# osmocom/osmo-gmr

Hardware: AMD Instinct MI355X
Metric: Mbursts/s demod+Viterbi (and IQ Msamp/s), 1/2/4/8 MI355X (higher is better)
Workload: dtype f32+i32

## Files before the change

osmo-gmr_amd/csrc/conv_k5_12.h:

```cpp
#pragma once
#include "l1_codes.h"
#include "rx4_operands.h"
#include "wave_ops.h"

namespace gmr1 {

__constant__ StepTable c_steps = make_steps();
__device__ const Rx4Steps4 g_steps4 = make_steps4(make_steps());

struct CostTable { uint32_t a[512], b[512]; };
static constexpr CostTable make_cost()
{
	CostTable t{};
	for (int idx = 0; idx < 512; idx++) {
		int v = (int)(int8_t)(uint8_t)(idx & 255);
		if (idx & 256)
			v = (int)(int8_t)(uint8_t)(-v);
		const int e0 = v - 127, e1 = v + 127;
		const uint32_t c0 = v ? (uint32_t)((e0 * e0) >> 9) : 0u;
		const uint32_t c1 = v ? (uint32_t)((e1 * e1) >> 9) : 0u;
		t.a[idx] = c0 | (c0 << 8) | (c1 << 16) | (c1 << 24);
		t.b[idx] = c0 | (c1 << 8) | (c0 << 16) | (c1 << 24);
	}
	return t;
}
__constant__ CostTable c_cost = make_cost();

static constexpr CostTable make_cost_acc()
{
	CostTable t{};
	for (int idx = 0; idx < 512; idx++) {
		int v = (int)(int8_t)(uint8_t)(idx & 255);
		if (idx & 256)
			v = (int)(int8_t)(uint8_t)(-v);
		const uint32_t c0 = v < 0 ? (uint32_t)(-v) : 0u;
		const uint32_t c1 = v > 0 ? (uint32_t)v : 0u;
		t.a[idx] = c0 | (c0 << 8) | (c1 << 16) | (c1 << 24);
		t.b[idx] = c0 | (c1 << 8) | (c0 << 16) | (c1 << 24);
	}
	return t;
}
__constant__ CostTable c_cost_acc = make_cost_acc();
constexpr uint32_t kAccLeadK5r2 = 127u * 2u * 5u / 2u;

struct SynTable { uint16_t s[208]; };
static constexpr SynTable make_syn()
{
	SynTable t{};
	for (int k = 0; k < 192; k++)
		t.s[k] = (uint16_t)l1c::crc_unit(l1c::kCrc16, k, 192);
	for (int i = 0; i < 16; i++)
		t.s[192 + i] = (uint16_t)(1u << (15 - i));
	return t;
}
__constant__ SynTable c_syn = make_syn();

struct SynRows { uint32_t w[16][8]; };
static constexpr SynRows make_syn_rows()
{
	const SynTable t = make_syn();
	SynRows r{};
	for (int loc = 0; loc < 16; loc++)
		for (int q = 0; q < 13; q++)
			r.w[loc][q >> 1] |= (uint32_t)t.s[13 * loc + q] << (16 * (q & 1));
	return r;
}
__constant__ __attribute__((aligned(16))) SynRows c_syn_rows = make_syn_rows();

struct SbLut { uint16_t v[1024]; };
static constexpr SbLut make_sb_lut()
{
	SbLut t{};
	for (int k = 0; k < 1024; k++) {
		int q = 2 * k + 1;
		if (q > 1024)
			q -= 2048;
		const int n = (q + 256 + 2048) / 512 - 4;
		const int dlq = 512 * n - q;
		const int adl = dlq < 0 ? -dlq : dlq;
		const int dq = (adl + 2) / 4;
		const unsigned sp = (unsigned)n & 3u;
		const unsigned neg = dlq < 0 ? 1u : 0u;
		const bool f0 = ((sp ^ neg ^ 1u) & 1u) != 0;
		const int m_near = 127 - dq, m_far = 127 - (dq >> 1);
		int v0 = f0 ? m_near : m_far;
		int v1 = f0 ? m_far : m_near;
		if (sp >> 1)
			v0 = -v0;
		if ((sp ^ (sp >> 1)) & 1u)
			v1 = -v1;
		t.v[k] = (uint16_t)(((unsigned)v0 & 0xffu) | (((unsigned)v1 & 0xffu) << 8));
	}
	return t;
}
__device__ __attribute__((aligned(16))) const SbLut g_sb_lut = make_sb_lut();
constexpr int kSbLutBytes = 2048;

static constexpr SbLut make_sb_lut1()
{
	SbLut t{};
	for (int k = 0; k < 1024; k++) {
		int q = 2 * k + 1;
		if (q > 1024)
			q -= 2048;
		const int n = (q + 512 + 2048) / 1024 - 2;
		const int dlq = 1024 * n - q;
		const int adl = dlq < 0 ? -dlq : dlq;
		const int dq = (adl + 4) / 8;
		const unsigned sp = (unsigned)n & 1u;
		const int v0 = sp ? -(127 - dq) : (127 - dq);
		t.v[k] = (uint16_t)((unsigned)v0 & 0xffu);
	}
	return t;
}
__device__ __attribute__((aligned(16))) const SbLut g_sb_lut1 = make_sb_lut1();

__device__ __forceinline__ uint32_t out_k5_12(uint32_t s, uint32_t b)
{
	constexpr uint32_t g0 = l1c::kK5_12[0], g1 = l1c::kK5_12[1];
	uint32_t reg = (s << 1) | b;
	return ((uint32_t)(__popc(reg & g0) & 1) << 1) | (uint32_t)(__popc(reg & g1) & 1);
}
__device__ __forceinline__ uint32_t rotl4(uint32_t x, int r) { return ((x << r) | (x >> (4 - r))) & 15u; }

template <bool ACC = false>
__device__ __forceinline__ void branch_metrics_k5_12(const int8_t *__restrict__ eb, int chain,
                                                     uint32_t *__restrict__ bm, int lane)
{
	const CostTable &ct = ACC ? c_cost_acc : c_cost;
	for (int k = lane; k < kSteps12; k += 64) {
		const uint32_t st = c_steps.w[chain][k];
		const uint32_t ia = (uint32_t)(uint8_t)eb[st & 0x3ffu] | ((st >> 2) & 0x100u);
		const uint32_t ib = (uint32_t)(uint8_t)eb[(st >> 16) & 0x3ffu] | ((st >> 18) & 0x100u);
		bm[k] = ct.a[ia] + ct.b[ib];
	}
}

template <bool ACC, class Steps>
__device__ __forceinline__ void branch_metrics4_k5_12_from(const int8_t *__restrict__ eb, int eb_stride, int row_ok,
                                                           int row_chain, uint32_t *__restrict__ bm, int lane, Steps steps)
{
	const CostTable &ct = ACC ? c_cost_acc : c_cost;
	uint32_t st[2][4];
#pragma unroll
	for (int c = 0; c < 2; c++)
#pragma unroll
		for (int it = 0; it < 4; it++)
			st[c][it] = steps(c, it);
	uint32_t ia[4][4], ib[4][4];
#pragma unroll
	for (int q = 0; q < 4; q++) {
		const bool ch = ((row_chain >> q) & 1) != 0;
		const int8_t *e = eb + q * eb_stride;
#pragma unroll
		for (int it = 0; it < 4; it++) {
			const uint32_t s = ch ? st[1][it] : st[0][it];
			ia[q][it] = (uint32_t)(uint8_t)e[s & 0x3ffu] | ((s >> 2) & 0x100u);
			ib[q][it] = (uint32_t)(uint8_t)e[(s >> 16) & 0x3ffu] | ((s >> 18) & 0x100u);
		}
	}
	uint32_t va[4][4], vb[4][4];
#pragma unroll
	for (int q = 0; q < 4; q++)
#pragma unroll
		for (int it = 0; it < 4; it++) {
			va[q][it] = ct.a[ia[q][it]];
			vb[q][it] = ct.b[ib[q][it]];
		}
#pragma unroll
	for (int q = 0; q < 4; q++) {
		const bool ok = ((row_ok >> q) & 1) != 0;
#pragma unroll
		for (int it = 0; it < 4; it++) {
			const int k = lane + 64 * it;
			if (k < kSteps12)
				bm[q * kSteps12 + k] = ok ? va[q][it] + vb[q][it] : 0u;
		}
	}
}

template <bool ACC = false>
__device__ __forceinline__ void branch_metrics4_k5_12(const int8_t *__restrict__ eb, int eb_stride, int row_ok,
                                                      int row_chain, uint32_t *__restrict__ bm, int lane)
{
	branch_metrics4_k5_12_from<ACC>(eb, eb_stride, row_ok, row_chain, bm, lane, [&](int c, int it) -> uint32_t {
		const int k = lane + 64 * it;
		return k < kSteps12 ? c_steps.w[c][k] : 0u;
	});
}

template <bool ACC = false>
__device__ __forceinline__ void branch_metrics4_k5_12(const int8_t *__restrict__ eb, int eb_stride, int row_ok,
                                                      int row_chain, uint32_t *__restrict__ bm, int lane,
                                                      const uint4 st0, const uint4 st1)
{
	branch_metrics4_k5_12_from<ACC>(eb, eb_stride, row_ok, row_chain, bm, lane, [&](int c, int it) -> uint32_t {
		const uint4 v = c ? st1 : st0;
		return it == 0 ? v.x : (it == 1 ? v.y : (it == 2 ? v.z : v.w));
	});
}

constexpr uint32_t kSentinel = 0xF0000000u;

struct DecTable { uint32_t v[16]; };
static constexpr uint32_t dec_out(uint32_t s, uint32_t b)
{
	return l1c::conv_word(l1c::kK5_12, (s << 1) | b);
}
static constexpr uint32_t dec_state(uint32_t loc, int ph)
{
	uint32_t c[4] = {0, 0, 0, 0};
	c[0] = (loc >> 3) & 1u;
	uint32_t x = loc & 7u;
	c[1] = (x >> 2) & 1u;
	x ^= c[1] ? 7u : 0u;
	c[2] = (x >> 1) & 1u;
	c[3] = x & 1u;
	uint32_t sp = 0;
	for (int i = 0; i < 4; i++)
		sp |= c[(3 - i + ph) & 3] << i;
	return sp;
}
static constexpr DecTable make_dec()
{
	DecTable t{};
	for (uint32_t loc = 0; loc < 16; loc++) {
		uint32_t e = 0;
		for (int ph = 0; ph < 4; ph++) {
			const uint32_t sp = dec_state(loc, ph);
			const uint32_t b = sp >> 3;
			e |= dec_out(sp, b) << (2 * ph);
			e |= dec_out(sp, b ^ 1u) << (8 + 2 * ph);
			for (int j = ph; j < 16; j += 4)
				e |= b << (16 + j);
		}
		t.v[loc] = e;
	}
	return t;
}
static constexpr bool dec_exchange_holds()
{
	const DecTable t = make_dec();
	const uint32_t mask[4] = {8u, 7u, 2u, 1u};
	for (uint32_t loc = 0; loc < 16; loc++)
		for (int ph = 0; ph < 4; ph++) {
			const uint32_t sp = dec_state(loc, ph);
			const uint32_t partner_into_mine = dec_out(sp ^ 8u, sp >> 3);
			if (dec_state(loc ^ mask[ph], ph) != (sp ^ 8u))
				return false;
			if (((t.v[loc ^ mask[ph]] >> (8 + 2 * ph)) & 3u) != partner_into_mine)
				return false;
			if (((t.v[loc] >> (8 + 2 * ph)) & 3u) != partner_into_mine)
// ... 374 lines not shown
```

osmo-gmr_amd/csrc/rx4_operands.h:

```cpp
#pragma once
#include <stdint.h>

#include "gmr1_dev.h"
#include "l1_codes.h"

namespace gmr1 {

static constexpr int kSteps12 = 212;

struct StepTable { uint32_t w[2][kSteps12]; };
static constexpr StepTable make_steps()
{
	StepTable t{};
	const auto scr = l1c::scramble_seq<448>();
	for (int chain = 0; chain < 2; chain++) {
		const int off = chain ? 4 : 0;
		for (int k = 0; k < kSteps12; k++) {
			uint32_t w = 0;
			for (int j = 0; j < 2; j++) {
				const int kc = 2 * k + j;
				const int ei = l1c::intra_pos(53, kc) + off;
				w |= ((uint32_t)ei | (scr.bit[ei] ? 0x400u : 0u)) << (16 * j);
			}
			t.w[chain][k] = w;
// ... 7 lines not shown
struct alignas(16) Rx4Steps4 { uint32_t w[2][64][4]; };
static constexpr Rx4Steps4 make_steps4(const StepTable &st)
{
	Rx4Steps4 t{};
	for (int chain = 0; chain < 2; chain++)
		for (int lane = 0; lane < 64; lane++)
			for (int it = 0; it < 4; it++) {
				const int k = lane + 64 * it;
				t.w[chain][lane][it] = k < kSteps12 ? st.w[chain][k] : 0u;
			}
	return t;
}

struct alignas(8) Rx4Ord4 { int16_t v[2][64][4]; };
inline void make_ord4(const DevBurst types[kNumTypes], Rx4Ord4 *out)
{
	for (int kind = 0; kind < 2; kind++) {
		const DevBurst &bt = types[kRx4Type[kind]];
		for (int lane = 0; lane < 64; lane++)
			for (int r = 0; r < 4; r++) {
				const int i = lane + 64 * r;
				out->v[kind][lane][r] = (i < bt.len && i < kMaxLen) ? bt.ord_of_sym[i] : (int16_t)-1;
			}
	}
}

inline bool rx4_ord4_matches(const DevBurst types[kNumTypes], const Rx4Ord4 &o)
{
	for (int kind = 0; kind < 2; kind++) {
		const DevBurst &bt = types[kRx4Type[kind]];
		if (bt.len > 256)
			return false;
		for (int lane = 0; lane < 64; lane++)
			for (int r = 0; r < 4; r++) {
				const int i = lane + 64 * r;
				if (o.v[kind][lane][r] != (i < bt.len ? bt.ord_of_sym[i] : (int16_t)-1))
					return false;
			}
	}
	return true;
}
inline bool rx4_steps4_matches(const StepTable &st, const Rx4Steps4 &s)
{
	for (int chain = 0; chain < 2; chain++)
		for (int lane = 0; lane < 64; lane++)
			for (int it = 0; it < 4; it++) {
				const int k = lane + 64 * it;
				if (s.w[chain][lane][it] != (k < kSteps12 ? st.w[chain][k] : 0u))
					return false;
			}
	return true;
}

}
```

osmo-gmr_amd/csrc/rx_kernels.hip:

```cpp
#include <mutex>
#include <type_traits>

#include "gmr1_dev.h"
#include "tch3_body.h"
#include "wave_ops.h"
#include "fast_math.h"

namespace gmr1 {
__constant__ DevBurst c_types[kNumTypes];
}

#include "conv_k5_12.h"
#include "rx_window.h"

namespace gmr1 {

__device__ Rx4Ord4 g_ord4;

#include "rx_one.h"

__device__ __forceinline__ float2 sync_coef0(const DevBurst &bt, int n, int sps, float fs)
{
	const int nch = bt.n_chunks[0];
	int ch = 0, base = 0, cum = 0;
// ... 360 lines not shown
	const DevBurst &bt = c_types[kind ? GMR1_HIP_DC6 : GMR1_HIP_BCCH];
	const int w = in_len - 234 * sps + 1;
	const float2 *__restrict__ in = a.iq + off;
	constexpr int NFULL = (SPS == 4 && NPL == 16) ? 15 : -1;
	constexpr int SIT = SPS == 4 ? 2 : 4;
	float2 wv[NPL];
	float2 sv[3][SIT];
	window_fetch<NPL, NFULL>(in, in_len, lane, wv);
#pragma unroll
	for (int c = 0; c < 3; c++) {
		const int wl = F::clen(bt, kind, c) * sps + w - 1;
		const float2 *__restrict__ src = in + F::cpos(bt, c) * sps;
#pragma unroll
		for (int h = 0; h < SIT; h++) {
			const int sidx = lane + 64 * h;
			sv[c][h] = sidx < wl ? src[sidx] : make_float2(0.f, 0.f);
		}
	}
	if (win) {
#pragma unroll
		for (int k = 0; k < NPL; k++)
			win[lane + 64 * k] = wv[k];
	}
	float avr, avi, inv;
	window_stats<NPL, NFULL>(wv, in_len, lane, avr, avi, inv);
	const float e = window_energy_regs<NPL>(wv, in_len, lane);
	int wb = 0;
#pragma unroll
	for (int c = 0; c < 3; c++) {
		const int wl = F::clen(bt, kind, c) * sps + w - 1;
#pragma unroll
		for (int h = 0; h < SIT; h++) {
			const int sidx = lane + 64 * h;
			if (sidx < wl) {
				const v2f nv = ((v2f){sv[c][h].x, sv[c][h].y} - (v2f){avr, avi}) * (v2f){inv, inv};
				hx[wb + sidx] = make_float2(nv.x, nv.y);
			}
		}
		wb += wl;
	}
	if (lane == 0) {
		hs[0] = avr;
		hs[1] = avi;
		hs[2] = inv;
		hs[3] = e;
	}
}

struct Rx4Cfg {
	static constexpr int NPL = 16, SPS = 4;
	static constexpr bool LAT = false, GEN = false, FAC = false, ACC = false, EN = true, PL = false;
	static constexpr int EBROW = 432, PART = 0;
	static constexpr bool EARLY = false;
};
template <int NPL_, int SPS_, bool ACC_, bool EN_, bool PL_ = false, bool EARLY_ = false>
struct CfgBatch : Rx4Cfg {
	static constexpr int NPL = NPL_, SPS = SPS_;
	static constexpr bool ACC = ACC_, EN = EN_, PL = PL_, EARLY = EARLY_;
};
template <int NPL_, int SPS_, bool FAC_>
struct CfgDemod : Rx4Cfg {
	static constexpr int NPL = NPL_, SPS = SPS_;
	static constexpr bool GEN = true, FAC = FAC_;
};
struct CfgTch3Front : Rx4Cfg {
	static constexpr int NPL = 8, SPS = 4, EBROW = 216;
	static constexpr bool GEN = true;
};
template <int NPL_, int SPS_, bool ACC_, int PART_ = 0>
struct CfgLoop : Rx4Cfg {
	static constexpr int NPL = NPL_, SPS = SPS_, PART = PART_;
	static constexpr bool LAT = true, ACC = ACC_;
};

#ifndef GMR1_EXP_RX4_TOUCH
#define GMR1_EXP_RX4_TOUCH 0
#endif

template <class P>
struct Rx4Switches : P {
	static constexpr bool SMALL = P::GEN && P::NPL == 8;
	static_assert(!P::FAC || SMALL, "the two-sequence variant builds on the small generic one");
	static_assert(!P::PL || (P::SPS == 4 && !P::GEN && !P::LAT && !P::EN), "the planar layout exists for the fused batch kernel at sps 4");
	static_assert(P::PART == 0 || P::LAT, "only the receive loop's burst is cut in two");
	static constexpr bool PREFETCH_NEXT = P::GEN || P::LAT;
	static constexpr int NSYM = SMALL ? 2 : 4;
	static constexpr int NCHK = SMALL ? 1 : 3;
	static constexpr int NSH = SMALL ? 1 : 2;
	static constexpr bool UB_OVER = !P::LAT && !P::GEN;
	static constexpr bool QL = !P::GEN && !P::LAT && !P::EN && P::SPS == 4 && P::NPL == 16;
	static constexpr bool QX = QL && !P::PL;
	static_assert(!P::PL || QL, "the planar layout exists for the fused batch kernel");
	static constexpr bool AHEAD = P::EARLY && QX;
	static constexpr int TOUCH = AHEAD ? GMR1_EXP_RX4_TOUCH : 0;
	static constexpr bool H_ROW = AHEAD, ONE_LOAD = AHEAD;
	static constexpr bool OPS_AHEAD = AHEAD;
};

constexpr int kRx4StepsAt = 1;

template <class Cfg>
__device__ __forceinline__ void rx4_body(const RxArgs &a, const RxIo io, int stage_samples, int cw, int g0, int n_end,
                                         unsigned char *__restrict__ lds_raw, int lane, LatPre<Cfg::NPL, Cfg::SPS> *pre = nullptr)
{
	typedef Rx4Switches<Cfg> C;
	constexpr int NPL = C::NPL, SPS = C::SPS, EBROW = C::EBROW, PART = C::PART;
	constexpr bool LAT = C::LAT, GEN = C::GEN, FAC = C::FAC, ACC = C::ACC, EN = C::EN, PL = C::PL;
	constexpr bool SMALL = C::SMALL, QL = C::QL, QX = C::QX, PREFETCH_NEXT = C::PREFETCH_NEXT, UB_OVER = C::UB_OVER;
	constexpr int NSYM = C::NSYM, NCHK = C::NCHK, NSH = C::NSH;
	constexpr int TOUCH = C::TOUCH;
	constexpr bool AHEAD = C::AHEAD, H_ROW = C::H_ROW, OPS_AHEAD = C::OPS_AHEAD;
	const int row = lane >> 4, col = lane & 15;
	const int sps = SPS ? SPS : a.sps;
	const int cwh = FAC ? cw / 2 : cw;
	size_t off[4];
	lds4_layout(stage_samples, cw, off, GEN, UB_OVER, EBROW);
	Lds4 L;
	L.x = reinterpret_cast<float2 *>(lds_raw + off[0]);
	L.corr = reinterpret_cast<float *>(lds_raw + off[1]);
	L.coef = reinterpret_cast<float2 *>(lds_raw + off[2]);
	L.eb = reinterpret_cast<int8_t *>(lds_raw + off[3]);
	L.bm = reinterpret_cast<uint32_t *>(lds_raw + off[0]);
	L.surv = reinterpret_cast<uint64_t *>(lds_raw + off[3]);
	L.ubits = reinterpret_cast<uint32_t *>(lds_raw + off[0] + (UB_OVER ? 0 : 4 * kSteps12 * 4));

	const int g_row = g0 + row;
	const bool row_live = g_row < n_end;

	float avr_r = 0.f, avi_r = 0.f;
	const float2 *xst_lat = L.x;

	float th_q[QX ? 4 : 1][4];
	uint32_t zm_q = 0xff000000u;
	float2 xs_q[2] = {make_float2(0.f, 0.f), make_float2(0.f, 0.f)};
	float inv_r = 1.0f;
	auto op_kind = [&](int g) -> int {
		if constexpr (LAT && PART != 0) return 0; else return io.kind[g] ? 1 : 0;
	};
	auto op_fsh = [&](int g) -> float {
		if constexpr (LAT && PART != 0) return pre->b_fsh; else return io.freq_shift ? io.freq_shift[g] : 0.0f;
	};
	auto op_off = [&](int g) -> uint64_t {
		if constexpr (LAT && PART != 0) return pre->b_off; else return io.offset[g];
	};
	int kind_s[4] = {0, 0, 0, 0};
	uint64_t off_s[4] = {0, 0, 0, 0};
	float fsh_s[4] = {0.f, 0.f, 0.f, 0.f};
	if constexpr (AHEAD) {
		if (g0 < n_end) {
			int kv[4];
			uint64_t ov[4];
			float fv[4];
#pragma unroll
			for (int q = 0; q < 4; q++) {
				const int gq = g0 + q < n_end ? g0 + q : g0;
				kv[q] = op_kind(gq);
				ov[q] = op_off(gq);
				fv[q] = op_fsh(gq);
			}
#pragma unroll
			for (int q = 0; q < 4; q++) {
				kind_s[q] = __builtin_amdgcn_readfirstlane(kv[q]);
				off_s[q] = (uint64_t)(uint32_t)__builtin_amdgcn_readfirstlane((int)(uint32_t)ov[q]) |
				           ((uint64_t)(uint32_t)__builtin_amdgcn_readfirstlane((int)(uint32_t)(ov[q] >> 32)) << 32);
				fsh_s[q] = __builtin_bit_cast(float, __builtin_amdgcn_readfirstlane(__builtin_bit_cast(int, fv[q])));
			}
		}
	}
	float2 wv_own[NPL];
	bool co_on = false;
	int co_p = 0;
	if constexpr (PART == 2)
		GMR1_STAMP(14);
	else
		GMR1_STAMP(0);
	if constexpr (PART != 2) {
	if constexpr (SMALL) {
		const DevBurst &bt = c_types[a.fixed_type];
		const int in_len = __builtin_amdgcn_readfirstlane(a.in_len[0]);
		const int w = in_len - bt.len * sps + 1;
		const int tl = bt.sync_tl[0];
		const int len0 = bt.sync[0][0].len;
		const int wl = len0 * sps + w - 1;
		const int gq = row_live ? g_row : g0;
		const float2 *__restrict__ in = a.iq + io.offset[gq];
		const float fsh = io.freq_shift ? io.freq_shift[gq] : 0.0f;
		const float fs = (fsh - bt.rotation) / (float)sps;
		float2 *xs = reinterpret_cast<float2 *>(lds_raw) + row * 64;
		L.corr = reinterpret_cast<float *>(lds_raw + 2048);
		float2 *coef = reinterpret_cast<float2 *>(lds_raw + 4096) + row * 16;
		float2 sv[4];
		{
			const float2 *__restrict__ src = in + bt.sync[0][0].pos * sps;
#pragma unroll
			for (int h = 0; h < 4; h++) {
				const int sidx = col + 16 * h;
				sv[h] = sidx < wl ? src[sidx] : make_float2(0.f, 0.f);
			}
		}
		const int nit = in_len >> 4, rem = in_len & 15;
		const bool want_en = io.energy != nullptr;
		v2f s2 = {0.f, 0.f}, q2 = {0.f, 0.f};
#pragma unroll 8
		for (int t = 0; t < nit; t++) {
			const float2 x = in[col + 16 * t];
			s2 += (v2f){x.x, x.y};
			q2 = __builtin_elementwise_fma((v2f){x.x, x.y}, (v2f){x.x, x.y}, q2);
		}
		if (col < rem) {
			const float2 x = in[col + 16 * nit];
			s2 += (v2f){x.x, x.y};
			q2 = __builtin_elementwise_fma((v2f){x.x, x.y}, (v2f){x.x, x.y}, q2);
		}
		float en = 0.f;
		if (want_en) {
			const int bd = in_len >> 5;
			for (int idx = col; idx < in_len; idx += 16)
				if (idx >= bd && idx < in_len - bd) {
					const float2 x = in[idx];
					en = fmaf(x.x, x.x, fmaf(x.y, x.y, en));
				}
// ... 845 lines not shown
				const float pr = (chn[0] == c ? t0[0].x : 0.f) + (chn[1] == c ? t0[1].x : 0.f);
				const float pi = (chn[0] == c ? t0[0].y : 0.f) + (chn[1] == c ? t0[1].y : 0.f);
				sumr[c] = row_sum(pr);
				sumi[c] = row_sum(pi);
			}
			float f = 0.f;
#pragma unroll
			for (int i = 1; i < NCS; i++) {
				if (i < nch_r) {
					const float ppos = (float)F::cpos(bt_r, i - 1) + (float)F::clen(bt_r, kind_r, i - 1) / 2.0f;
					const float cpos = (float)F::cpos(bt_r, i) + (float)F::clen(bt_r, kind_r, i) / 2.0f;
					const float re = sumr[i] * sumr[i - 1] - sumi[i] * (-sumi[i - 1]);
					const float im = sumr[i] * (-sumi[i - 1]) + sumi[i] * sumr[i - 1];
					f += atan2_fast(im, re) / (cpos - ppos);
				}
			}
			ffe_r = f / (float)(nch_r - 1);
		}
		float tr = 0.f, ti = 0.f;
#pragma unroll
		for (int h = 0; h < NSH; h++) {
			float2 tt = t0[h];
			if (ffe_r != 0.0f) {
				float s, c;
				sincos_fast(-ffe_r * (float)spos[h], s, c);
				tt = cmul(tt, make_float2(c, s));
			}
			tr += tt.x;
			ti += tt.y;
		}
		psi_r = atan2_fast(row_sum(ti), row_sum(tr));
	}
	if constexpr (PART != 2) {
	GMR1_STAMP(4);
	if (a.dbg_stop == 5) return;

	if (col == 0 && row_live && (PART != 1 || io.rv)) {
		const int rv = found_r ? 0 : -1;
		io.rv[g_row] = rv;
		if (io.sync_id) io.sync_id[g_row] = found_r ? sid_r : -1;
		if (io.toa) io.toa[g_row] = found_r ? toa_r : 0.f;
		if (io.freq_err) io.freq_err[g_row] = found_r ? ffe_r : 0.f;
	}
	}
	if constexpr (PART == 1) {
		auto first_f = [](float v) { return __builtin_bit_cast(float, __builtin_amdgcn_readfirstlane(__builtin_bit_cast(int, v))); };
		pre->out = {__builtin_amdgcn_readfirstlane(found_r ? 1 : 0), __builtin_amdgcn_readfirstlane(d_r), __builtin_amdgcn_readfirstlane(sid_r),
		            first_f(found_r ? toa_r : 0.f), first_f(found_r ? ffe_r : 0.f), first_f(psi_r), first_f(avr_r), first_f(avi_r)};
		if (lane == 0)
			*pre->cut = {found_r ? 1 : 0, d_r, sid_r, toa_r, ffe_r, psi_r, avr_r, avi_r};
		return;
	}

	const unsigned char *lut = lds_raw + (GEN ? 4 * EBROW : 0);
	uint2 ord4_q[4] = {};
	uint4 st4[2] = {};
	if constexpr (LAT) {
		lut = pre->lut;
		WSYNC();
	} else {
		unsigned char *const lutw = lds_raw + (GEN ? 4 * EBROW : 0);
		const uint4 *__restrict__ lut_src = reinterpret_cast<const uint4 *>(FAC ? g_sb_lut1.v : g_sb_lut.v);
		const uint4 lut_a = lut_src[lane], lut_b = lut_src[lane + 64];
		if constexpr (OPS_AHEAD) {
			const uint2 *__restrict__ ord_src = reinterpret_cast<const uint2 *>(g_ord4.v);
#pragma unroll
			for (int q = 0; q < 4; q++)
				ord4_q[q] = ord_src[(uint32_t)((kind_s[q] ? 64 : 0) + lane)];
		}
		WSYNC();
		reinterpret_cast<uint4 *>(lutw)[lane] = lut_a;
		reinterpret_cast<uint4 *>(lutw)[lane + 64] = lut_b;
		WSYNC();
	}

	int row_ok = 0, row_chain = 0;
	Sym4 nxt1, nxt2;
	if constexpr (!QX) { nxt1 = first; nxt2 = second; }
#pragma unroll
	for (int q = 3; q >= 0; q--) {
		const int g = g0 + q;
		if constexpr (OPS_AHEAD) {
			if (q == kRx4StepsAt) {
				const uint4 *__restrict__ st_src = reinterpret_cast<const uint4 *>(g_steps4.w);
#pragma unroll
				for (int c = 0; c < 2; c++)
					st4[c] = st_src[(uint32_t)(64 * c + lane)];
			}
		}
		Sym4 cur;
		if constexpr (LAT) {
			if (q != 0)
				continue;
			cur = first;
		} else if constexpr (QX) {
			cur.ok = 0;
#pragma unroll
			for (int r = 0; r < NSYM; r++) cur.x[r] = make_float2(0.f, 0.f);
		} else {
			cur = nxt1;
			nxt1 = nxt2;
			fetch(q - 2, nxt2);
		}
		if (g >= n_end)
			continue;
		const int src = 16 * q;
		const bool hit = QX && __builtin_amdgcn_readlane((int)hit_r, src) != 0;
		if constexpr (QX) {
			if (!hit && __builtin_amdgcn_readlane((int)found_r, src) != 0) {
				if (q == first_q)
					cur = first;
				else
					fetch(q, cur);
			}
		}
		const bool found = __builtin_amdgcn_readlane((int)found_r, src) != 0;
		const int kind = __builtin_amdgcn_readlane(kind_r, src);
		const int type = GEN ? a.fixed_type : (kind ? GMR1_HIP_DC6 : GMR1_HIP_BCCH);
		const DevBurst &bt = c_types[type];
		const int d = __builtin_amdgcn_readlane(d_r, src);
		const float fs = lane_val(fs_r, src);
		const float rps = -lane_val(ffe_r, src);
		const float psi = lane_val(psi_r, src);
		const float avr = lane_val(avr_r, src), avi = lane_val(avi_r, src);
		const int blen = F::len(bt), nbits = F::nbits(bt);
		float *gss = io.ssyms ? io.ssyms + (size_t)g * a.ssyms_stride : nullptr;
		int8_t *eb = L.eb + q * (GEN ? EBROW : 432);
		row_chain |= kind << q;
		if (!found) {
			if (io.ebits)
				for (int i = lane; i < a.ebits_stride; i += 64)
					if (!GEN || i < bt.ebits)
						io.ebits[(size_t)g * a.ebits_stride + i] = 0;
			if constexpr (GEN)
				for (int i = lane; i < EBROW / 4; i += 64)
					reinterpret_cast<uint32_t *>(eb)[i] = 0;
			if (gss)
				for (int i = lane; i < blen; i += 64)
					gss[i] = 0.f;
			continue;
		}
		row_ok |= 1 << q;
		int ordv[NSYM];
#pragma unroll
		for (int r = 0; r < NSYM; r++) {
			const int i = lane + 64 * r;
			if constexpr (OPS_AHEAD) {
				const uint32_t pair = r < 2 ? ord4_q[q].x : ord4_q[q].y;
				ordv[r] = (r & 1) ? (int)pair >> 16 : (int)(pair << 16) >> 16;
			} else {
				ordv[r] = i < blen ? bt.ord_of_sym[i] : -1;
			}
		}
		const float kInv2Pi = 0.159154943091895336f;
		const float At = (fs * (float)sps + rps) * kInv2Pi;
		float Bt = (fs * (float)d - psi) * kInv2Pi;
		Bt -= rintf(Bt);
		const float A2 = At * 2048.0f, B2 = Bt * 2048.0f;
		const float scale = (float)(1 << nbits);
		float2 mref = make_float2(avr, avi);
		if constexpr (GEN) {
			if (gss)
				mref = window_mean_serial(a.iq + io.offset[g], a.in_len[0]);
		}
#pragma unroll
		for (int r = 0; r < NSYM; r++) {
			const int i = lane + 64 * r;
			if (i >= blen)
				continue;
			float2 x = cur.x[r];
			x.x -= avr;
			x.y -= avi;
			float at;
			bool zero;
			if (QX && hit) {
				at = th_q[QX ? q : 0][r];
				zero = ((zm_q >> (4 * q + r)) & 1u) != 0;
			} else {
				at = atan2_turns(x.y, x.x);
				zero = !(cur.ok & (1 << r)) || (x.x == 0.0f && x.y == 0.0f);
			}
			const float th2 = fmaf(A2, (float)i, fmaf(at, 2048.0f, B2));
			if (gss) {
				float th = th2 * (1.0f / 2048.0f);
				bool zero_ss = zero;
				if constexpr (GEN) {
					const float xr = cur.x[r].x - mref.x, xi = cur.x[r].y - mref.y;
					th = fmaf(A2, (float)i, fmaf(atan2_turns(xi, xr), 2048.0f, B2)) * (1.0f / 2048.0f);
					zero_ss = !(cur.ok & (1 << r)) || (xr == 0.0f && xi == 0.0f);
				}
				th -= rintf(th);
				gss[i] = zero_ss ? 0.0f : th * scale;
			}
			const int ord = ordv[r];
			if (ord >= 0) {
				int cell;
				asm("v_cvt_flr_i32_f32 %0, %1" : "=v"(cell) : "v"(th2));
				cell = zero ? 0 : (cell & 2046);
				if constexpr (FAC)
					eb[ord] = (int8_t)lut[cell];
				else
					*reinterpret_cast<uint16_t *>(eb + 2 * ord) = *reinterpret_cast<const uint16_t *>(lut + cell);
			}
		}
		if (io.ebits) {
			WSYNC();
			const int neb = bt.ebits;
			int8_t *ge = io.ebits + (size_t)g * a.ebits_stride;
			for (int i = lane; i < a.ebits_stride; i += 64)
				if (!GEN || i < neb)
					ge[i] = i < neb ? eb[i] : (int8_t)0;
		}
	}
	if (GEN || (a.dbg_stop && a.dbg_stop < 7))
		return;
	GMR1_STAMP(5);

	WSYNC();
	DecPre dpre;
	if constexpr (LAT) {
		const int chain = row_chain & 1;
		const bool ok = (row_ok & 1) != 0;
#pragma unroll
		for (int it = 0; it < 4; it++) {
			const int k = lane + 64 * it;
			if (k < kSteps12) {
				const uint32_t stw = pre->steps[chain * kSteps12 + k];
				const uint32_t ia = (uint32_t)(uint8_t)L.eb[stw & 0x3ffu] | ((stw >> 2) & 0x100u);
				const uint32_t ib = (uint32_t)(uint8_t)L.eb[(stw >> 16) & 0x3ffu] | ((stw >> 18) & 0x100u);
				lat_expand_step(pre->vtab, k, ok ? pre->cost_a[ia] + pre->cost_b[ib] : 0u);
			}
		}
		dpre.dc = pre->dc; dpre.sy0 = pre->sy0; dpre.sy1 = pre->sy1;
#ifdef GMR1_HIP_PROFILE
		dpre.stamp = io.stamp;
#endif
	} else if constexpr (OPS_AHEAD) {
		dpre.dc = c_dec.v[col];
		dpre.sy0 = *reinterpret_cast<const uint4 *>(&c_syn_rows.w[col][0]);
		dpre.sy1 = *reinterpret_cast<const uint4 *>(&c_syn_rows.w[col][4]);
		branch_metrics4_k5_12<ACC>(L.eb, 432, row_ok, row_chain, L.bm, lane, st4[0], st4[1]);
	} else {
		branch_metrics4_k5_12<ACC>(L.eb, 432, row_ok, row_chain, L.bm, lane);
	}
	WSYNC();
	GMR1_STAMP(6);
	if (a.dbg_stop == 7)
		return;
	if constexpr (PART == 2)
		return;
	uint32_t syn, fae;
	if constexpr (LAT)
		decode1_k5_12_lat<ACC>(pre->vtab, L.surv, L.ubits, lane, syn, fae, &dpre);
	else
		decode4_k5_12<ACC>(L.bm, L.surv, L.ubits, lane, syn, fae, OPS_AHEAD ? &dpre : nullptr);
	GMR1_STAMP(7);
	if (col == 0 && row_live) {
		if ((row_ok >> row) & 1) {
			store_l2(io.l2 + (size_t)g_row * 24, L.ubits + row * 8);
			io.crc[g_row] = syn ? 1 : 0;
			io.conv[g_row] = (int32_t)fae;
		} else {
			uint32_t *l2w = reinterpret_cast<uint32_t *>(io.l2 + (size_t)g_row * 24);
#pragma unroll
			for (int i = 0; i < 6; i++)
				l2w[i] = 0;
			io.crc[g_row] = -1;
			io.conv[g_row] = 0;
		}
	}
}

#ifndef GMR1_EXP_RX4_WAVES
#define GMR1_EXP_RX4_WAVES 6
#endif
template <int NPL, int SPS, bool EN = false>
constexpr int kRx4Waves = NPL > 16 ? 3 : ((SPS == 4 && !EN) ? GMR1_EXP_RX4_WAVES : 5);

template <int NPL, int SPS, bool ACC = false, bool EN = false, bool PL = false>
__global__ __launch_bounds__(64) __attribute__((amdgpu_waves_per_eu(kRx4Waves<NPL, SPS, EN>, kRx4Waves<NPL, SPS, EN>)))
void k_rx4(RxArgs a, int stage_samples, int cw, int bpw)
{
	extern __shared__ __align__(16) unsigned char lds_raw[];
	int g0 = blockIdx.x * bpw;
	int n_end = min(a.n, g0 + bpw);
	if (EN && a.seg_count) {
		int sg = g0 / a.seg_stride;
		int lo = 0;
		if (a.seg_first) {
			if (a.seg_groups > 0) {
				sg = (int)blockIdx.x / a.seg_groups;
				lo = (a.seg_first[sg] + 3) & ~3;
				g0 = sg * a.seg_stride + lo + ((int)blockIdx.x % a.seg_groups) * bpw;
			} else {
				lo = (a.seg_first[sg] + 3) & ~3;
			}
		}
		const int base = sg * a.seg_stride;
		n_end = min(min(a.n, g0 + bpw), base + min(a.seg_count[sg], a.seg_stride));
		if (g0 >= n_end || g0 < base + lo)
			return;
	}
	const RxIo io = {
#ifdef GMR1_HIP_PROFILE
	                 nullptr,
#endif
	                 a.offset, a.kind, a.freq_shift, a.l2, a.crc, a.conv, a.rv, a.sync_id, a.toa, a.freq_err, a.energy,
	                 a.ebits, a.ssyms};
	rx4_body<CfgBatch<NPL, SPS, ACC, EN, PL, true>>(a, io, stage_samples, cw, g0, n_end, lds_raw, (int)threadIdx.x);
}

template <int NPL, int SPS, bool FAC = false>
__global__ __launch_bounds__(64) void k_rx4g(RxArgs a, int stage_samples, int cw)
{
	extern __shared__ __align__(16) unsigned char lds_raw[];
	const int g0 = blockIdx.x * 4;
	const RxIo io = {
#ifdef GMR1_HIP_PROFILE
	                 nullptr,
#endif
	                 a.offset, nullptr, a.freq_shift, nullptr, nullptr, nullptr, a.rv, a.sync_id, a.toa, a.freq_err, a.energy,
	                 a.ebits, a.ssyms};
	rx4_body<CfgDemod<NPL, SPS, FAC>>(a, io, stage_samples, cw, g0, min(a.n, g0 + 4), lds_raw, (int)threadIdx.x);
}

template <bool ACC>
constexpr int kRx4gTch3Waves = 7;
template <bool ACC>
__global__ __launch_bounds__(64) __attribute__((amdgpu_waves_per_eu(kRx4gTch3Waves<ACC>, kRx4gTch3Waves<ACC>))) void k_rx4g_tch3(RxArgs a, Tch3Args t, int stage_samples, int cw)
{
	extern __shared__ __align__(16) unsigned char lds_raw[];
	const int g0 = blockIdx.x * 4;
	const int lane = (int)threadIdx.x;
	const int n_end = min(a.n, g0 + 4);
	const RxIo io = {
#ifdef GMR1_HIP_PROFILE
	                 nullptr,
#endif
	                 a.offset, nullptr, a.freq_shift, nullptr, nullptr, nullptr, a.rv, a.sync_id, a.toa, a.freq_err, a.energy,
	                 a.ebits, a.ssyms};
	constexpr int kRow = 216;
	static_assert(CfgTch3Front::EBROW == kRow, "the body's soft-bit rows are the decoder's");
	rx4_body<CfgTch3Front>(a, io, stage_samples, cw, g0, n_end, lds_raw, lane);
	t3::Tch3Lds *S = reinterpret_cast<t3::Tch3Lds *>(lds_raw + 4 * kRow);
	WSYNC();
	t3::tch3_fill_locof(S, lane);
	if (lane < 4)
		*reinterpret_cast<uint32_t *>(lds_raw + lane * kRow + 212) = 0;
	t3::Tch3Lane lc;
	t3::tch3_lane(lc, S, lane);
	WSYNC();
	for (int q = 0; q < 4 && g0 + q < n_end; q++) {
		t3::tch3_burst<ACC>(t, g0 + q, lane, reinterpret_cast<const int8_t *>(lds_raw + q * kRow), S, lc);
		WSYNC();
	}
}

#include "rx_small_kernels.h"

template <int NPL, int SPS>
static hipError_t launch_rx_t(const RxArgs &a, bool decode, int max_in_len, int max_len, hipStream_t stream)
{
	size_t off[3];
	const size_t lds = lds_layout(max_in_len, max_len, decode, off);
	if (decode) {
		const bool sliced = a.seg_first && a.seg_groups > 0 && a.seg_stride > 0;
		const int grid = sliced ? (a.n / a.seg_stride) * a.seg_groups : (a.n + 3) / 4;
		if (a.impl == 1 || NPL > 32) {
			if (a.conv_acc)
				hipLaunchKernelGGL((k_rx<NPL, SPS, true, true>), dim3(grid), dim3(64), lds, stream, a, max_in_len, max_len);
			else
				hipLaunchKernelGGL((k_rx<NPL, SPS, true>), dim3(grid), dim3(64), lds, stream, a, max_in_len, max_len);
		} else if constexpr (NPL <= 32) {
			const int cw = (max_len + 15) & ~15;
			size_t off4[4];
			const size_t lds4 = lds4_layout(a.stage_samples, cw, off4, false, true);
			static size_t pad = (size_t)-1;
			if (pad == (size_t)-1) {
				const char *e = profile_env("GMR1_HIP_LDS_PAD");
				pad = e ? (size_t)atoi(e) : 0;
			}
			static int bpw_force = -1;
			if (bpw_force < 0) {
				const char *e = profile_env("GMR1_HIP_RX_BPW");
				bpw_force = e ? atoi(e) : 0;
			}
			const int bpw = sliced ? 4 : (bpw_force == 1 || bpw_force == 4 ? bpw_force : (a.n <= 4096 ? 1 : 4));
			const int grid4 = sliced ? (a.n / a.seg_stride) * a.seg_groups : (a.n + bpw - 1) / bpw;
			const bool en = a.energy != nullptr || a.seg_count != nullptr;
			if (a.plane_stride) {
				if constexpr (NPL == 16 && SPS == 4) {
					if (en)
						return hipErrorInvalidValue;
					if (a.conv_acc)
						hipLaunchKernelGGL((k_rx4<16, 4, true, false, true>), dim3(grid4), dim3(64), lds4 + pad, stream, a, a.stage_samples, cw, bpw);
					else
						hipLaunchKernelGGL((k_rx4<16, 4, false, false, true>), dim3(grid4), dim3(64), lds4 + pad, stream, a, a.stage_samples, cw, bpw);
				} else
					return hipErrorInvalidValue;
			} else
			if (a.conv_acc) {
				if (en)
					hipLaunchKernelGGL((k_rx4<NPL, SPS, true, true>), dim3(grid4), dim3(64), lds4 + pad, stream, a, a.stage_samples, cw, bpw);
				else
					hipLaunchKernelGGL((k_rx4<NPL, SPS, true, false>), dim3(grid4), dim3(64), lds4 + pad, stream, a, a.stage_samples, cw, bpw);
			} else {
				if (en)
					hipLaunchKernelGGL((k_rx4<NPL, SPS, false, true>), dim3(grid4), dim3(64), lds4 + pad, stream, a, a.stage_samples, cw, bpw);
				else
					hipLaunchKernelGGL((k_rx4<NPL, SPS, false, false>), dim3(grid4), dim3(64), lds4 + pad, stream, a, a.stage_samples, cw, bpw);
			}
		}
	} else {
		hipLaunchKernelGGL((k_rx<NPL, SPS, false>), dim3(a.n), dim3(64), lds, stream, a, max_in_len, max_len);
	}
	return hipGetLastError();
}

hipError_t launch_rx(const RxArgs &a, bool decode, int max_in_len, hipStream_t stream)
{
	if (a.n <= 0)
		return hipSuccess;
	if (max_in_len > kMaxInLen)
		return hipErrorInvalidValue;
	const int w_demod = a.in_len[0] - a.ssyms_stride * a.sps + 1;
	const int max_len = decode ? (20 * a.sps + 1) : (w_demod > kMaxWindow ? w_demod : kMaxWindow);
	if (!decode && (a.impl == 2 || a.impl == 3 || a.impl == 4) && a.sps == 4 && max_in_len <= 1024) {
		const int cw1 = (a.in_len[0] - a.ssyms_stride * 4 + 1 + 15) & ~15;
		const int cw = a.impl == 4 ? 2 * cw1 : cw1;
		size_t off4[4];
		const size_t lds4 = lds4_layout(a.stage_samples, cw, off4, true);
		const int grid4 = (a.n + 3) / 4;
		if (a.impl == 4)
			hipLaunchKernelGGL((k_rx4g<8, 4, true>), dim3(grid4), dim3(64), lds4, stream, a, a.stage_samples, cw);
		else if (a.impl == 3)
			hipLaunchKernelGGL((k_rx4g<8, 4>), dim3(grid4), dim3(64), lds4, stream, a, a.stage_samples, cw);
		else
			hipLaunchKernelGGL((k_rx4g<16, 4>), dim3(grid4), dim3(64), lds4, stream, a, a.stage_samples, cw);
		return hipGetLastError();
	}
	if (max_in_len <= 1024) {
		if (a.sps == 4)
			return launch_rx_t<16, 4>(a, decode, max_in_len, max_len, stream);
		return launch_rx_t<16, 0>(a, decode, max_in_len, max_len, stream);
	}
	if (max_in_len <= 2048) {
		if (a.sps == 4)
			return launch_rx_t<32, 4>(a, decode, max_in_len, max_len, stream);
		return launch_rx_t<32, 0>(a, decode, max_in_len, max_len, stream);
	}
	return launch_rx_t<64, 0>(a, decode, max_in_len, max_len, stream);
}
// ... 55 lines not shown
```

Baseline: 475.9.

## Stage soft-bit LUT and cost tables in LDS via LDS-DMA for batch rx4 kernel

Adds an LT variant of the batch rx4 kernel with a fixed LDS carve. The soft-bit LUT is loaded into LDS with global_load_lds instead of being built per block. The ordering tables are fetched per kind rather than per row. The cost tables are folded to a single 256-entry table, with the B variant derived through a byte permute and the sign flip applied arithmetically. That folded table can be DMA'd into LDS so branch metrics read from LDS rather than constant memory. This trades extra vmcnt waits and a new launch path (only when the carve fits and energy is off) for fewer table-construction and constant-cache lookups.

```diff
diff --git a/osmo-gmr_amd/csrc/conv_k5_12.h b/osmo-gmr_amd/csrc/conv_k5_12.h
--- a/osmo-gmr_amd/csrc/conv_k5_12.h
+++ b/osmo-gmr_amd/csrc/conv_k5_12.h
@@ -8,39 +8,10 @@
 __constant__ StepTable c_steps = make_steps();
 __device__ const Rx4Steps4 g_steps4 = make_steps4(make_steps());
 
-struct CostTable { uint32_t a[512], b[512]; };
-static constexpr CostTable make_cost()
-{
-	CostTable t{};
-	for (int idx = 0; idx < 512; idx++) {
-		int v = (int)(int8_t)(uint8_t)(idx & 255);
-		if (idx & 256)
-			v = (int)(int8_t)(uint8_t)(-v);
-		const int e0 = v - 127, e1 = v + 127;
-		const uint32_t c0 = v ? (uint32_t)((e0 * e0) >> 9) : 0u;
-		const uint32_t c1 = v ? (uint32_t)((e1 * e1) >> 9) : 0u;
-		t.a[idx] = c0 | (c0 << 8) | (c1 << 16) | (c1 << 24);
-		t.b[idx] = c0 | (c1 << 8) | (c0 << 16) | (c1 << 24);
-	}
-	return t;
-}
 __constant__ CostTable c_cost = make_cost();
 
-static constexpr CostTable make_cost_acc()
-{
-	CostTable t{};
-	for (int idx = 0; idx < 512; idx++) {
-		int v = (int)(int8_t)(uint8_t)(idx & 255);
-		if (idx & 256)
-			v = (int)(int8_t)(uint8_t)(-v);
-		const uint32_t c0 = v < 0 ? (uint32_t)(-v) : 0u;
-		const uint32_t c1 = v > 0 ? (uint32_t)v : 0u;
-		t.a[idx] = c0 | (c0 << 8) | (c1 << 16) | (c1 << 24);
-		t.b[idx] = c0 | (c1 << 8) | (c0 << 16) | (c1 << 24);
-	}
-	return t;
-}
 __constant__ CostTable c_cost_acc = make_cost_acc();
+__device__ const Rx4CostFold g_cost_fold = make_cost_fold(make_cost(), make_cost_acc());
 constexpr uint32_t kAccLeadK5r2 = 127u * 2u * 5u / 2u;
 
 struct SynTable { uint16_t s[208]; };
@@ -67,34 +38,7 @@
 }
 __constant__ __attribute__((aligned(16))) SynRows c_syn_rows = make_syn_rows();
 
-struct SbLut { uint16_t v[1024]; };
-static constexpr SbLut make_sb_lut()
-{
-	SbLut t{};
-	for (int k = 0; k < 1024; k++) {
-		int q = 2 * k + 1;
-		if (q > 1024)
-			q -= 2048;
-		const int n = (q + 256 + 2048) / 512 - 4;
-		const int dlq = 512 * n - q;
-		const int adl = dlq < 0 ? -dlq : dlq;
-		const int dq = (adl + 2) / 4;
-		const unsigned sp = (unsigned)n & 3u;
-		const unsigned neg = dlq < 0 ? 1u : 0u;
-		const bool f0 = ((sp ^ neg ^ 1u) & 1u) != 0;
-		const int m_near = 127 - dq, m_far = 127 - (dq >> 1);
-		int v0 = f0 ? m_near : m_far;
-		int v1 = f0 ? m_far : m_near;
-		if (sp >> 1)
-			v0 = -v0;
-		if ((sp ^ (sp >> 1)) & 1u)
-			v1 = -v1;
-		t.v[k] = (uint16_t)(((unsigned)v0 & 0xffu) | (((unsigned)v1 & 0xffu) << 8));
-	}
-	return t;
-}
 __device__ __attribute__((aligned(16))) const SbLut g_sb_lut = make_sb_lut();
-constexpr int kSbLutBytes = 2048;
 
 static constexpr SbLut make_sb_lut1()
 {
@@ -136,9 +80,10 @@
 	}
 }
 
-template <bool ACC, class Steps>
+template <bool ACC, class Steps, bool FOLD = false>
 __device__ __forceinline__ void branch_metrics4_k5_12_from(const int8_t *__restrict__ eb, int eb_stride, int row_ok,
-                                                           int row_chain, uint32_t *__restrict__ bm, int lane, Steps steps)
+                                                           int row_chain, uint32_t *__restrict__ bm, int lane, Steps steps,
+                                                           const uint32_t *fold = nullptr)
 {
 	const CostTable &ct = ACC ? c_cost_acc : c_cost;
 	uint32_t st[2][4];
@@ -147,6 +92,35 @@
 #pragma unroll
 		for (int it = 0; it < 4; it++)
 			st[c][it] = steps(c, it);
+	if constexpr (FOLD) {
+#pragma unroll
+		for (int q = 0; q < 4; q++) {
+			const bool ch = ((row_chain >> q) & 1) != 0, ok = ((row_ok >> q) & 1) != 0;
+			const int8_t *e = eb + q * eb_stride;
+			uint32_t ua[4], ub[4];
+#pragma unroll
+			for (int it = 0; it < 4; it++) {
+				const uint32_t s = ch ? st[1][it] : st[0][it];
+				ua[it] = (uint32_t)(uint8_t)e[s & 0x3ffu];
+				ub[it] = (uint32_t)(uint8_t)e[(s >> 16) & 0x3ffu];
+			}
+			uint32_t wa[4], wb[4];
+#pragma unroll
+			for (int it = 0; it < 4; it++) {
+				const uint32_t s = ch ? st[1][it] : st[0][it];
+				const uint32_t ma = (uint32_t)((int32_t)(s << 21) >> 31), mb = (uint32_t)((int32_t)(s << 5) >> 31);
+				wa[it] = fold[((ua[it] ^ ma) - ma) & 0xffu];
+				wb[it] = fold[((ub[it] ^ mb) - mb) & 0xffu];
+			}
+#pragma unroll
+			for (int it = 0; it < 4; it++) {
+				const int k = lane + 64 * it;
+				if (k < kSteps12)
+					bm[q * kSteps12 + k] = ok ? wa[it] + __builtin_amdgcn_perm(wb[it], wb[it], kCostPermB) : 0u;
+			}
+		}
+		return;
+	}
 	uint32_t ia[4][4], ib[4][4];
 #pragma unroll
 	for (int q = 0; q < 4; q++) {
@@ -198,6 +172,18 @@
 		const uint4 v = c ? st1 : st0;
 		return it == 0 ? v.x : (it == 1 ? v.y : (it == 2 ? v.z : v.w));
 	});
+}
+
+template <bool ACC = false>
+__device__ __forceinline__ void branch_metrics4_k5_12_fold(const int8_t *__restrict__ eb, int eb_stride, int row_ok,
+                                                           int row_chain, uint32_t *__restrict__ bm, int lane,
+                                                           const uint4 st0, const uint4 st1, const uint32_t *fold)
+{
+	auto steps = [&](int c, int it) -> uint32_t {
+		const uint4 v = c ? st1 : st0;
+		return it == 0 ? v.x : (it == 1 ? v.y : (it == 2 ? v.z : v.w));
+	};
+	branch_metrics4_k5_12_from<ACC, decltype(steps), true>(eb, eb_stride, row_ok, row_chain, bm, lane, steps, fold);
 }
 
 constexpr uint32_t kSentinel = 0xF0000000u;
diff --git a/osmo-gmr_amd/csrc/rx4_operands.h b/osmo-gmr_amd/csrc/rx4_operands.h
--- a/osmo-gmr_amd/csrc/rx4_operands.h
+++ b/osmo-gmr_amd/csrc/rx4_operands.h
@@ -83,4 +83,98 @@
 	return true;
 }
 
+struct CostTable { uint32_t a[512], b[512]; };
+static constexpr CostTable make_cost()
+{
+	CostTable t{};
+	for (int idx = 0; idx < 512; idx++) {
+		int v = (int)(int8_t)(uint8_t)(idx & 255);
+		if (idx & 256)
+			v = (int)(int8_t)(uint8_t)(-v);
+		const int e0 = v - 127, e1 = v + 127;
+		const uint32_t c0 = v ? (uint32_t)((e0 * e0) >> 9) : 0u;
+		const uint32_t c1 = v ? (uint32_t)((e1 * e1) >> 9) : 0u;
+		t.a[idx] = c0 | (c0 << 8) | (c1 << 16) | (c1 << 24);
+		t.b[idx] = c0 | (c1 << 8) | (c0 << 16) | (c1 << 24);
+	}
+	return t;
 }
+
+static constexpr CostTable make_cost_acc()
+{
+	CostTable t{};
+	for (int idx = 0; idx < 512; idx++) {
+		int v = (int)(int8_t)(uint8_t)(idx & 255);
+		if (idx & 256)
+			v = (int)(int8_t)(uint8_t)(-v);
+		const uint32_t c0 = v < 0 ? (uint32_t)(-v) : 0u;
+		const uint32_t c1 = v > 0 ? (uint32_t)v : 0u;
+		t.a[idx] = c0 | (c0 << 8) | (c1 << 16) | (c1 << 24);
+		t.b[idx] = c0 | (c1 << 8) | (c0 << 16) | (c1 << 24);
+	}
+	return t;
+}
+
+struct alignas(16) Rx4CostFold { uint32_t a[2][256]; };
+constexpr uint32_t kCostPermB = 0x03010200u;
+static constexpr Rx4CostFold make_cost_fold(const CostTable &gen, const CostTable &acc)
+{
+	Rx4CostFold t{};
+	for (int idx = 0; idx < 256; idx++) {
+		t.a[0][idx] = gen.a[idx];
+		t.a[1][idx] = acc.a[idx];
+	}
+	return t;
+}
+static constexpr uint32_t cost_fold_index(int v, bool flip) { return (uint32_t)(uint8_t)(flip ? -v : v); }
+static constexpr uint32_t cost_fold_b(uint32_t a) { return (a & 0xff0000ffu) | ((a & 0x0000ff00u) << 8) | ((a & 0x00ff0000u) >> 8); }
+
+struct SbLut { uint16_t v[1024]; };
+static constexpr SbLut make_sb_lut()
+{
+	SbLut t{};
+	for (int k = 0; k < 1024; k++) {
+		int q = 2 * k + 1;
+		if (q > 1024)
+			q -= 2048;
+		const int n = (q + 256 + 2048) / 512 - 4;
+		const int dlq = 512 * n - q;
+		const int adl = dlq < 0 ? -dlq : dlq;
+		const int dq = (adl + 2) / 4;
+		const unsigned sp = (unsigned)n & 3u;
+		const unsigned neg = dlq < 0 ? 1u : 0u;
+		const bool f0 = ((sp ^ neg ^ 1u) & 1u) != 0;
+		const int m_near = 127 - dq, m_far = 127 - (dq >> 1);
+		int v0 = f0 ? m_near : m_far;
+		int v1 = f0 ? m_far : m_near;
+		if (sp >> 1)
+			v0 = -v0;
+		if ((sp ^ (sp >> 1)) & 1u)
+			v1 = -v1;
+		t.v[k] = (uint16_t)(((unsigned)v0 & 0xffu) | (((unsigned)v1 & 0xffu) << 8));
+	}
+	return t;
+}
+constexpr int kSbLutBytes = 2048;
+
+struct Rx4Region { uint32_t off, bytes; };
+struct Rx4LdsCarve {
+	static constexpr uint32_t kEb = 0, kCost = 4 * 432, kBm = kCost + 1024, kSbLut = 4352, kBytes = kSbLut + kSbLutBytes;
+	bool fits;
+	uint32_t bytes;
+	Rx4Region pass1, sb_lut, eb, cost, bm, surv, ubits;
+};
+static_assert(Rx4LdsCarve::kBm + 4 * kSteps12 * 4 <= Rx4LdsCarve::kBytes && Rx4LdsCarve::kBm % 16 == 0 &&
+              Rx4LdsCarve::kCost % 16 == 0 && Rx4LdsCarve::kSbLut % 16 == 0 && Rx4LdsCarve::kBytes % 1280 == 0,
+              "the metrics end inside the wave's LDS; what a 16-byte access or an LDS-DMA lands on is 16-byte aligned");
+constexpr Rx4LdsCarve rx4_lds_carve(int stage_samples, int cw)
+{
+	typedef Rx4LdsCarve C;
+	const uint64_t p1 = stage_samples < 0 || cw < 0 ? ~(uint64_t)0
+	                    : (((uint64_t)stage_samples * 8 + 15) & ~(uint64_t)15) + (((uint64_t)cw * 16 + 15) & ~(uint64_t)15) + 18 * 8;
+	const bool fits = p1 <= C::kSbLut;
+	return {fits, C::kBytes, {0, fits ? (uint32_t)p1 : 0u}, {C::kSbLut, (uint32_t)kSbLutBytes}, {C::kEb, 4 * 432},
+	        {C::kCost, 1024}, {C::kBm, 4 * kSteps12 * 4}, {C::kEb, 13 * 64 * 2}, {C::kBm, 4 * 8 * 4}};
+}
+
+}
diff --git a/osmo-gmr_amd/csrc/rx_kernels.hip b/osmo-gmr_amd/csrc/rx_kernels.hip
--- a/osmo-gmr_amd/csrc/rx_kernels.hip
+++ b/osmo-gmr_amd/csrc/rx_kernels.hip
@@ -436,11 +436,12 @@
 	static constexpr bool LAT = false, GEN = false, FAC = false, ACC = false, EN = true, PL = false;
 	static constexpr int EBROW = 432, PART = 0;
 	static constexpr bool EARLY = false;
+	static constexpr bool LT = false;
 };
-template <int NPL_, int SPS_, bool ACC_, bool EN_, bool PL_ = false, bool EARLY_ = false>
+template <int NPL_, int SPS_, bool ACC_, bool EN_, bool PL_ = false, bool EARLY_ = false, bool LT_ = false>
 struct CfgBatch : Rx4Cfg {
 	static constexpr int NPL = NPL_, SPS = SPS_;
-	static constexpr bool ACC = ACC_, EN = EN_, PL = PL_, EARLY = EARLY_;
+	static constexpr bool ACC = ACC_, EN = EN_, PL = PL_, EARLY = EARLY_, LT = LT_;
 };
 template <int NPL_, int SPS_, bool FAC_>
 struct CfgDemod : Rx4Cfg {
@@ -459,6 +460,22 @@
 
 #ifndef GMR1_EXP_RX4_TOUCH
 #define GMR1_EXP_RX4_TOUCH 0
+#endif
+
+#ifndef GMR1_EXP_RX4_LDS_TABLES
+#define GMR1_EXP_RX4_LDS_TABLES 1
+#endif
+#ifndef GMR1_EXP_RX4_STEPS_FRONT
+#define GMR1_EXP_RX4_STEPS_FRONT 0
+#endif
+#ifndef GMR1_EXP_RX4_ORD_LDS
+#define GMR1_EXP_RX4_ORD_LDS 0
+#endif
+#ifndef GMR1_EXP_RX4_STEPS_AT
+#define GMR1_EXP_RX4_STEPS_AT 1
+#endif
+#ifndef GMR1_EXP_RX4_COST_AT
+#define GMR1_EXP_RX4_COST_AT 1
 #endif
 
 template <class P>
@@ -479,6 +496,10 @@
 	static constexpr int TOUCH = AHEAD ? GMR1_EXP_RX4_TOUCH : 0;
 	static constexpr bool H_ROW = AHEAD, ONE_LOAD = AHEAD;
 	static constexpr bool OPS_AHEAD = AHEAD;
+	static constexpr bool LDS_TABLES = P::LT && OPS_AHEAD && GMR1_EXP_RX4_LDS_TABLES != 0;
+	static constexpr bool LDS_COST = LDS_TABLES && GMR1_EXP_RX4_LDS_TABLES >= 2;
+	static constexpr bool STEPS_FRONT = LDS_TABLES && GMR1_EXP_RX4_STEPS_FRONT != 0;
+	static_assert(!P::LT || OPS_AHEAD, "the tables in LDS are the early batch kernel's");
 };
 
 constexpr int kRx4StepsAt = 1;
@@ -494,6 +515,7 @@
 	constexpr int NSYM = C::NSYM, NCHK = C::NCHK, NSH = C::NSH;
 	constexpr int TOUCH = C::TOUCH;
 	constexpr bool AHEAD = C::AHEAD, H_ROW = C::H_ROW, OPS_AHEAD = C::OPS_AHEAD;
+	constexpr bool LDS_TABLES = C::LDS_TABLES, LDS_COST = C::LDS_COST, STEPS_FRONT = C::STEPS_FRONT;
 	const int row = lane >> 4, col = lane & 15;
 	const int sps = SPS ? SPS : a.sps;
 	const int cwh = FAC ? cw / 2 : cw;
@@ -507,6 +529,12 @@
 	L.bm = reinterpret_cast<uint32_t *>(lds_raw + off[0]);
 	L.surv = reinterpret_cast<uint64_t *>(lds_raw + off[3]);
 	L.ubits = reinterpret_cast<uint32_t *>(lds_raw + off[0] + (UB_OVER ? 0 : 4 * kSteps12 * 4));
+	if constexpr (LDS_TABLES) {
+		L.eb = reinterpret_cast<int8_t *>(lds_raw + Rx4LdsCarve::kEb);
+		L.surv = reinterpret_cast<uint64_t *>(lds_raw + Rx4LdsCarve::kEb);
+		L.bm = reinterpret_cast<uint32_t *>(lds_raw + Rx4LdsCarve::kBm);
+		L.ubits = reinterpret_cast<uint32_t *>(lds_raw + Rx4LdsCarve::kBm);
+	}
 
 	const int g_row = g0 + row;
 	const bool row_live = g_row < n_end;
@@ -551,6 +579,14 @@
 			}
 		}
 	}
+#if defined(__HIP_DEVICE_COMPILE__)
+	if constexpr (LDS_TABLES) {
+		typedef __attribute__((address_space(3))) void lds_void;
+		const unsigned char *src = reinterpret_cast<const unsigned char *>(g_sb_lut.v) + 16 * lane;
+		__builtin_amdgcn_global_load_lds(src, (lds_void *)(lds_raw + Rx4LdsCarve::kSbLut), 16, 0, 0);
+		__builtin_amdgcn_global_load_lds(src + 1024, (lds_void *)(lds_raw + Rx4LdsCarve::kSbLut + 1024), 16, 0, 0);
+	}
+#endif
 	float2 wv_own[NPL];
 	bool co_on = false;
 	int co_p = 0;
@@ -1502,11 +1538,42 @@
 		return;
 	}
 
-	const unsigned char *lut = lds_raw + (GEN ? 4 * EBROW : 0);
+	const unsigned char *lut = lds_raw + (LDS_TABLES ? Rx4LdsCarve::kSbLut : (GEN ? 4 * EBROW : 0));
 	uint2 ord4_q[4] = {};
 	uint4 st4[2] = {};
+	auto cost_dma = [&]() {
+#if defined(__HIP_DEVICE_COMPILE__)
+		typedef __attribute__((address_space(3))) void lds_void;
+		const unsigned char *src = reinterpret_cast<const unsigned char *>(g_cost_fold.a[ACC ? 1 : 0]) + (uint32_t)(16 * lane);
+		__builtin_amdgcn_global_load_lds(src, (lds_void *)(lds_raw + Rx4LdsCarve::kCost), 16, 0, 0);
+#endif
+	};
 	if constexpr (LAT) {
 		lut = pre->lut;
+		WSYNC();
+	} else if constexpr (LDS_TABLES) {
+		WSYNC();
+		if constexpr (LDS_COST && GMR1_EXP_RX4_COST_AT < 0)
+			cost_dma();
+		if constexpr (GMR1_EXP_RX4_ORD_LDS) {
+#if defined(__HIP_DEVICE_COMPILE__)
+			typedef __attribute__((address_space(3))) void lds_void;
+			const unsigned char *src = reinterpret_cast<const unsigned char *>(g_ord4.v) + (uint32_t)(16 * lane);
+			__builtin_amdgcn_global_load_lds(src, (lds_void *)(lds_raw + Rx4LdsCarve::kBm), 16, 0, 0);
+#endif
+		} else {
+			const uint2 *__restrict__ ord_src = reinterpret_cast<const uint2 *>(g_ord4.v);
+#pragma unroll
+			for (int k = 0; k < 2; k++)
+				ord4_q[k] = ord_src[(uint32_t)(64 * k + lane)];
+		}
+		if constexpr (STEPS_FRONT) {
+			const uint4 *__restrict__ st_src = reinterpret_cast<const uint4 *>(g_steps4.w);
+#pragma unroll
+			for (int c = 0; c < 2; c++)
+				st4[c] = st_src[(uint32_t)(64 * c + lane)];
+		}
+		asm volatile("s_waitcnt vmcnt(0)" ::: "memory");
 		WSYNC();
 	} else {
 		unsigned char *const lutw = lds_raw + (GEN ? 4 * EBROW : 0);
@@ -1531,7 +1598,9 @@
 	for (int q = 3; q >= 0; q--) {
 		const int g = g0 + q;
 		if constexpr (OPS_AHEAD) {
-			if (q == kRx4StepsAt) {
+			if (LDS_COST && q == GMR1_EXP_RX4_COST_AT)
+				cost_dma();
+			if (!STEPS_FRONT && q == (LDS_TABLES ? GMR1_EXP_RX4_STEPS_AT : kRx4StepsAt)) {
 				const uint4 *__restrict__ st_src = reinterpret_cast<const uint4 *>(g_steps4.w);
 #pragma unroll
 				for (int c = 0; c < 2; c++)
@@ -1596,7 +1665,10 @@
 		for (int r = 0; r < NSYM; r++) {
 			const int i = lane + 64 * r;
 			if constexpr (OPS_AHEAD) {
-				const uint32_t pair = r < 2 ? ord4_q[q].x : ord4_q[q].y;
+				uint2 o4 = LDS_TABLES ? (kind_s[q] ? ord4_q[1] : ord4_q[0]) : ord4_q[q];
+				if constexpr (LDS_TABLES && GMR1_EXP_RX4_ORD_LDS)
+					o4 = *reinterpret_cast<const uint2 *>(lds_raw + Rx4LdsCarve::kBm + (kind_s[q] ? 512 : 0) + 8 * lane);
+				const uint32_t pair = r < 2 ? o4.x : o4.y;
 				ordv[r] = (r & 1) ? (int)pair >> 16 : (int)(pair << 16) >> 16;
 			} else {
 				ordv[r] = i < blen ? bt.ord_of_sym[i] : -1;
@@ -1666,6 +1738,8 @@
 		return;
 	GMR1_STAMP(5);
 
+	if constexpr (LDS_COST)
+		asm volatile("s_waitcnt vmcnt(0)" ::: "memory");
 	WSYNC();
 	DecPre dpre;
 	if constexpr (LAT) {
@@ -1689,7 +1763,11 @@
 		dpre.dc = c_dec.v[col];
 		dpre.sy0 = *reinterpret_cast<const uint4 *>(&c_syn_rows.w[col][0]);
 		dpre.sy1 = *reinterpret_cast<const uint4 *>(&c_syn_rows.w[col][4]);
-		branch_metrics4_k5_12<ACC>(L.eb, 432, row_ok, row_chain, L.bm, lane, st4[0], st4[1]);
+		if constexpr (LDS_COST)
+			branch_metrics4_k5_12_fold<ACC>(L.eb, 432, row_ok, row_chain, L.bm, lane, st4[0], st4[1],
+			                                reinterpret_cast<const uint32_t *>(lds_raw + Rx4LdsCarve::kCost));
+		else
+			branch_metrics4_k5_12<ACC>(L.eb, 432, row_ok, row_chain, L.bm, lane, st4[0], st4[1]);
 	} else {
 		branch_metrics4_k5_12<ACC>(L.eb, 432, row_ok, row_chain, L.bm, lane);
 	}
@@ -1727,7 +1805,7 @@
 template <int NPL, int SPS, bool EN = false>
 constexpr int kRx4Waves = NPL > 16 ? 3 : ((SPS == 4 && !EN) ? GMR1_EXP_RX4_WAVES : 5);
 
-template <int NPL, int SPS, bool ACC = false, bool EN = false, bool PL = false>
+template <int NPL, int SPS, bool ACC = false, bool EN = false, bool PL = false, bool LT = false>
 __global__ __launch_bounds__(64) __attribute__((amdgpu_waves_per_eu(kRx4Waves<NPL, SPS, EN>, kRx4Waves<NPL, SPS, EN>)))
 void k_rx4(RxArgs a, int stage_samples, int cw, int bpw)
 {
@@ -1757,7 +1835,7 @@
 #endif
 	                 a.offset, a.kind, a.freq_shift, a.l2, a.crc, a.conv, a.rv, a.sync_id, a.toa, a.freq_err, a.energy,
 	                 a.ebits, a.ssyms};
-	rx4_body<CfgBatch<NPL, SPS, ACC, EN, PL, true>>(a, io, stage_samples, cw, g0, n_end, lds_raw, (int)threadIdx.x);
+	rx4_body<CfgBatch<NPL, SPS, ACC, EN, PL, true, LT>>(a, io, stage_samples, cw, g0, n_end, lds_raw, (int)threadIdx.x);
 }
 
 template <int NPL, int SPS, bool FAC = false>
@@ -1848,6 +1926,14 @@
 						hipLaunchKernelGGL((k_rx4<16, 4, false, false, true>), dim3(grid4), dim3(64), lds4 + pad, stream, a, a.stage_samples, cw, bpw);
 				} else
 					return hipErrorInvalidValue;
+			} else if (NPL == 16 && SPS == 4 && !en && rx4_lds_carve(a.stage_samples, cw).fits) {
+				if constexpr (NPL == 16 && SPS == 4) {
+					const size_t ldst = rx4_lds_carve(a.stage_samples, cw).bytes;
+					if (a.conv_acc)
+						hipLaunchKernelGGL((k_rx4<16, 4, true, false, false, true>), dim3(grid4), dim3(64), ldst + pad, stream, a, a.stage_samples, cw, bpw);
+					else
+						hipLaunchKernelGGL((k_rx4<16, 4, false, false, false, true>), dim3(grid4), dim3(64), ldst + pad, stream, a, a.stage_samples, cw, bpw);
+				}
 			} else
 			if (a.conv_acc) {
 				if (en)
```

Result: no change. 479.3 (median of 2 runs) (+0.7%).
